# holuca/NeuralVolumetricReconstructionForMedicalImages

Measured on AMD Instinct MI355X. Metric: train rays/sec, chest 256^3 / 50 proj, higher is better.
Workload: dtype bf16; 1 GPU; chest_50.yaml: 256^3 volume, 50 cone-beam projections 512x512, hash L=16 T=2^19 C=2 (bf16 table), S=192, MLP 32-32-32-(64)-32-1, Adam lr 0.001; 1024 rays/step/GPU (reference n_rays=1024) = 1024 distinct valid pixels from one projection, drawn on the device inside the step; perturb=True; loss: chunk_sum (sum of 200-ray chunk means); the operating point that reaches 35 dB volume PSNR soonest (psnr.*; n_samples=192, parallelism=dp1

## Files before the change

include/naf_hip.h:

```cpp
#ifndef NAF_HIP_H
#define NAF_HIP_H

#include <stddef.h>
#include <stdint.h>

#ifdef __cplusplus
extern "C" {
#endif

typedef enum naf_status {
    NAF_OK = 0,
    NAF_ERR_INVALID_ARGUMENT = -1,
    NAF_ERR_UNSUPPORTED = -2,
    NAF_ERR_LAUNCH = -3
} naf_status;

typedef enum naf_dtype { NAF_F32 = 0, NAF_F16 = 1, NAF_BF16 = 2 } naf_dtype;

typedef enum naf_layout {
    NAF_LAYOUT_LBC = 0,
    NAF_LAYOUT_BLC = 1
} naf_layout;

const char *naf_last_error(void);
// ... 57 lines not shown
    float bound;
    uint32_t L, C, H;
    int32_t table_dtype;
    int32_t mlp_precision;
    int32_t last_activation;
    uint64_t seed;
    uint32_t ray_index_base;
    uint32_t log2_hashmap_size;
    int32_t scatter_mode;
    uint32_t flags;
} naf_render_cfg;

#define NAF_SCATTER_AUTO 0
#define NAF_SCATTER_ATOMIC 1
#define NAF_SCATTER_BINNED 2

#define NAF_CFG_PER_LEVEL_LAUNCHES 1u
#define NAF_CFG_EXPLICIT_DEPTHS 2u
#define NAF_CFG_LEVELS_INTERLEAVED 4u

#define NAF_CFG_FORWARD_FUSED 8u
#define NAF_CFG_ENCODE_TWO_GATHERS 32u
#define NAF_CFG_BACKWARD_ONE_WAVE_PER_SIMD 128u
#define NAF_CFG_ENCODE_LEVEL_MAJOR 256u
#define NAF_CFG_ENCODE_WINDOWS 64u
#define NAF_CFG_FUSED_STORE_FEATURES 16u
#define NAF_CFG_ENCODE_GROUPS_2 512u
#define NAF_CFG_ENCODE_GROUPS_4 1024u
#define NAF_CFG_MIN_BUCKETS_SHIFT 13u
#define NAF_CFG_MIN_BUCKETS_MASK (3u << NAF_CFG_MIN_BUCKETS_SHIFT)
#define NAF_CFG_SCATTER_PAIR12 2048u
#define NAF_CFG_LEVELS_GATHER_PASS 32768u
#define NAF_CFG_MLP_TWO_KERNELS 65536u
#define NAF_CFG_TEST_TINY_BLOCKS 4096u


int naf_scatter_overflow_count(const naf_render_cfg *cfg, uint64_t n_points, const void *workspace, uint32_t *count_host);

int naf_scatter_overflow_levels(const naf_render_cfg *cfg, uint64_t n_points, const void *workspace, uint32_t *counts_host);

size_t naf_render_workspace_bytes(const naf_render_cfg *cfg, uint64_t n_points);

size_t naf_forward_workspace_bytes(const naf_render_cfg *cfg, uint64_t n_points);

int naf_render_forward(const float *rays, const float *t_rand, const void *embeddings, const int32_t *offsets,
                       const float *mlp, float *acc, uint32_t n_rays, const naf_render_cfg *cfg, void *workspace,
                       void *stream);

int naf_render_forward_samples(const float *rays, const float *t_rand, const void *embeddings, const int32_t *offsets,
                               const float *mlp, float *acc, float *sigma, float *optical_depth, uint32_t n_rays,
                               const naf_render_cfg *cfg, void *workspace, void *stream);

int naf_render_backward(const float *rays, const float *t_rand, const float *grad_acc, const void *embeddings,
                        const int32_t *offsets, const float *mlp, float *grad_embeddings, float *grad_mlp, uint32_t n_rays,
                        const naf_render_cfg *cfg, void *workspace, int features_valid, void *stream);

int naf_render_train(const float *rays, const float *t_rand, const float *target, const float *ray_weight,
                     const void *embeddings, const int32_t *offsets, const float *mlp, float *acc,
                     float *grad_embeddings, float *grad_mlp, float *loss_out, uint32_t n_rays,
                     const naf_render_cfg *cfg, void *workspace, void *stream);

#define NAF_MAX_GRAD_BUCKETS 16
typedef struct naf_grad_buckets {
    uint32_t n_buckets;
    uint32_t level_begin[NAF_MAX_GRAD_BUCKETS];
    uint32_t level_end[NAF_MAX_GRAD_BUCKETS];
// ... 83 lines not shown
```

neuralvolumetricreconstructionformedicalimages_amd/_abi.py:

```python
from __future__ import annotations

import ctypes
import os

import torch

from . import build as _build

F32, F16, BF16 = 0, 1, 2
LAYOUT_LBC, LAYOUT_BLC = 0, 1
MLP_PARAMS = 4225
SCATTER_AUTO, SCATTER_ATOMIC, SCATTER_BINNED = 0, 1, 2
CFG_PER_LEVEL_LAUNCHES = 1
CFG_EXPLICIT_DEPTHS = 2
CFG_LEVELS_INTERLEAVED = 4
CFG_FORWARD_FUSED = 8
CFG_FUSED_STORE_FEATURES = 16
CFG_ENCODE_TWO_GATHERS = 32
CFG_ENCODE_WINDOWS = 64
CFG_BACKWARD_ONE_WAVE_PER_SIMD = 128
CFG_ENCODE_LEVEL_MAJOR = 256
CFG_ENCODE_GROUPS_2 = 512
CFG_ENCODE_GROUPS_4 = 1024
CFG_SCATTER_PAIR12 = 2048
CFG_TEST_TINY_BLOCKS = 4096
CFG_LEVELS_GATHER_PASS = 32768
CFG_MLP_TWO_KERNELS = 65536
CFG_MIN_BUCKETS_SHIFT = 13
GRAD_INPUTS_NONE, GRAD_INPUTS_EXACT, GRAD_INPUTS_REFERENCE = 0, 1, 2

_DTYPE_CODE = {torch.float32: F32, torch.float16: F16, torch.bfloat16: BF16}
_lib = None


class RenderCfg(ctypes.Structure):
    _fields_ = [
        ("n_samples", ctypes.c_uint32), ("perturb", ctypes.c_int32), ("bound", ctypes.c_float),
        ("L", ctypes.c_uint32), ("C", ctypes.c_uint32), ("H", ctypes.c_uint32),
        ("table_dtype", ctypes.c_int32), ("mlp_precision", ctypes.c_int32), ("last_activation", ctypes.c_int32),
        ("seed", ctypes.c_uint64), ("ray_index_base", ctypes.c_uint32), ("log2_hashmap_size", ctypes.c_uint32),
        ("scatter_mode", ctypes.c_int32), ("flags", ctypes.c_uint32),
    ]


MAX_GRAD_BUCKETS = 16


class GradBuckets(ctypes.Structure):
    _fields_ = [
        ("n_buckets", ctypes.c_uint32), ("level_begin", ctypes.c_uint32 * MAX_GRAD_BUCKETS),
        ("level_end", ctypes.c_uint32 * MAX_GRAD_BUCKETS), ("ready", ctypes.c_void_p * MAX_GRAD_BUCKETS),
        ("mlp_ready", ctypes.c_void_p),
    ]


MAX_DRAW_SEGMENTS = 16


class TableAdam(ctypes.Structure):
    _fields_ = [
# ... 150 lines not shown
```

neuralvolumetricreconstructionformedicalimages_amd/csrc/render_fused.hip:

```cpp
#include <algorithm>
#include <cmath>
#include <cstdio>
#include <cstring>
#include <type_traits>

#include "naf_host.h"
#include "hash_kernels.h"
#include "encode_kernel.h"
#include "field_mlp.h"
#include "field_mlp16.h"
#include "fused_forward.h"
#include "mlp_slabs.h"
#include "scatter_binned.h"
#include "scatter_v2.h"
#include "scatter_host.h"

namespace naf {

template <uint32_t kBytes> struct RawWord;
template <> struct RawWord<2> { typedef uint16_t type; };
template <> struct RawWord<4> { typedef uint32_t type; };
template <> struct RawWord<8> { typedef uint2 type; };
template <> struct RawWord<16> { typedef uint4 type; };

// ... 1107 lines not shown
    if (int rc = check_launch("mlp_backward_kernel")) return rc;
    if (ex.after_backward != nullptr && hipEventRecord(ex.after_backward, s) != hipSuccess) return fail(NAF_ERR_LAUNCH, "mlp backward: cannot record the event");
    return run_mlp_grad_reduce(slabs, grid, grad_mlp, loss_out, with_loss, madam, gmax_bits, ex, s);
}

static bool adam_tail_possible(const naf_render_cfg *cfg, const Workspace &w, uint32_t lv_begin, uint32_t lv_end) {
    if (!w.binned || per_level_launches(cfg)) return false;
    const uint32_t NB = 1u << w.plan.log2_nb;
    for (uint32_t l0 = lv_begin; l0 < lv_end; l0 += w.plan.levels_per_pass)
        if (reducer_split(NB, std::min(w.plan.levels_per_pass, lv_end - l0)) != 1u) return false;
    return true;
}

#ifndef NAF_V2_LV_FEW
#define NAF_V2_LV_FEW 4u
#endif
struct FxRecords {
    using Rec = PairFx;
    static constexpr uint32_t kThreads = 512u, kPoints = 2u, kLvMany = 16u, kLvFew = NAF_V2_LV_FEW;
    static constexpr bool kHasBig = true;
    const SrcRays &src;
    const void *dfeat;
    uint32_t B;
    DrawJob *next_draw;
    const GradBlocks *from_blocks;

    template <bool kFromBlocks>
    static auto bin_kernel_of(bool big, bool nb64, bool many) {
        constexpr uint32_t NT = kThreads;
        return big ? (many ? scatter_bin2_kernel<2u * NT, kLvMany, 0u, kFromBlocks> : scatter_bin2_kernel<2u * NT, kLvFew, 0u, kFromBlocks>)
                   : nb64 ? (many ? scatter_bin2_kernel<NT, kLvMany, 6u, kFromBlocks> : scatter_bin2_kernel<NT, kLvFew, 6u, kFromBlocks>)
                          : (many ? scatter_bin2_kernel<NT, kLvMany, 0u, kFromBlocks> : scatter_bin2_kernel<NT, kLvFew, 0u, kFromBlocks>);
    }
    auto bin_kernel(const BinPlan &plan, bool big, bool many) const {
        const bool nb64 = plan.log2_nb == 6u;
        return from_blocks != nullptr ? bin_kernel_of<true>(big, nb64, many) : bin_kernel_of<false>(big, nb64, many);
    }
    auto reduce_kernel(const AdamTail *adam) const {
        const bool fast = adam != nullptr && adam->lp != nullptr;
        return adam == nullptr ? scatter_reduce2_kernel<false, false> : fast ? scatter_reduce2_kernel<true, true> : scatter_reduce2_kernel<true, false>;
    }
    uint32_t bin_lds(const BinPlan &plan) const {
        return (3u * (1u << plan.log2_nb) + 4u) * 4u + (plan.slots + 1u) * (uint32_t)sizeof(PairFx) + side_list_capacity(plan.slots) * 12u;
    }
    template <typename K>
    void launch_bin(K bin, dim3 grid, uint32_t threads, uint32_t lds, hipStream_t s, const BinPass &p) const {
        DrawJob dj{};
        if (next_draw != nullptr && next_draw->count != 0u) { dj = *next_draw; next_draw->count = 0u; }
        grid.x += (dj.count + threads - 1u) / threads;
        const GradBlocks gb = from_blocks != nullptr ? *from_blocks : GradBlocks{};
        hipLaunchKernelGGL(bin, grid, dim3(threads), lds, s, src, (const uint16_t *)dfeat, p.offsets, p.grad_table, (PairFx *)p.w.regions,
                           p.w.counts, p.w.overflow, B, p.H, p.l0, p.nl, p.plan, p.job, dj, gb);
    }
};

template <typename P, uint32_t C>
static int run_hash_backward_levels(const SrcRays &src, const void *dfeat, const int32_t *offsets, float *grad_table, uint32_t B,
                                    const naf_render_cfg *cfg, const Workspace &w, uint32_t lv_begin, uint32_t lv_end, hipStream_t s,
                                    const naf_grad_buckets *buckets = nullptr, const AdamTail *adam = nullptr, const SlabReduce *slab_job = nullptr,
                                    DrawJob *next_draw = nullptr, const GradBlocks *from_blocks = nullptr) {
    using FT = typename P::feat_t;
    if (from_blocks != nullptr && !(w.binned && scatter_v2(cfg))) return fail(NAF_ERR_LAUNCH, "hash backward: only the 8-byte-record scatter reads gradient blocks in place");
    if (w.binned) {
        if (scatter_v2(cfg)) {
            FxRecords fam{src, dfeat, B, next_draw, from_blocks};
            return launch_binned_scatter(fam, cfg, w.plan, w.bin, offsets, grad_table, lv_begin, lv_end, buckets, s, adam, slab_job);
        }
        if (cfg->mlp_precision == NAF_F32) {
            PairRecords<FT, C, SrcRays, PairF32<C>, 16u, true> fam{src, dfeat, B, B, 1u};
            return launch_binned_scatter(fam, cfg, w.plan, w.bin, offsets, grad_table, lv_begin, lv_end, buckets, s, adam, slab_job);
        }
        PairRecords<FT, C, SrcRays, PairBF16<C>, 16u, true> fam{src, dfeat, B, B, 1u};
        return launch_binned_scatter(fam, cfg, w.plan, w.bin, offsets, grad_table, lv_begin, lv_end, buckets, s, adam, slab_job);
    }
    if (adam != nullptr) return fail(NAF_ERR_LAUNCH, "hash backward: the Adam tail needs the binned scatter");
    if (per_level_launches(cfg)) {
        static const char *const names[32] = NAF_LEVEL_NAMES("hash_backward_kernel_L");
        for (uint32_t l = lv_begin; l < lv_end; ++l) {
            ProfScope prof_(level_name(names, l), s);
            hipLaunchKernelGGL((hash_backward_kernel<FT, 3, C, SrcRays>), dim3(hash_grid_x(B), 1), dim3(256), 0, s, src,
                               (const typename FT::store_t *)dfeat, offsets, grad_table, B, cfg->L, cfg->H, false, l);
        }
        return check_launch("hash_backward_kernel");
    }
    { ProfScope prof_("hash_backward_kernel", s); hipLaunchKernelGGL((hash_backward_kernel<FT, 3, C, SrcRays>), dim3(hash_grid_x(B), lv_end - lv_begin), dim3(256), 0, s, src,
// ... 238 lines not shown
    const uint32_t units = vec ? run / (uint32_t)(16u / sizeof(T)) : run;
    const uint32_t gx = std::max<uint32_t>(1u, std::min<uint32_t>((units + 1023u) / 1024u, std::max<uint32_t>(1u, 512u / (n_ranks * nl))));
    {
        ProfScope prof_("levels_gather_kernel", s);
        if (vec) hipLaunchKernelGGL((levels_gather_kernel<T, true>), dim3(gx, n_ranks * nl), dim3(256), 0, s, (const unsigned char *)blocks, block_stride, (T *)w.dfeat, n_ranks, nl, run, lv_begin, gmax);
        else hipLaunchKernelGGL((levels_gather_kernel<T, false>), dim3(gx, n_ranks * nl), dim3(256), 0, s, (const unsigned char *)blocks, block_stride, (T *)w.dfeat, n_ranks, nl, run, lv_begin, gmax);
    }
    if (int rc = check_launch("levels_gather_kernel")) return rc;
    return run_hash_backward_levels<P, C>(src, w.dfeat, offsets, grad_emb, B, cfg, w, lv_begin, lv_end, s, nullptr, fuse ? &tail : nullptr, nullptr);
}

#define NAF_DISPATCH_PC(FN, ...)                                                                      \
    do {                                                                                              \
        if (cfg->mlp_precision == NAF_F32) {                                                          \
            switch (cfg->C) {                                                                         \
                case 1: return FN<PrecF32, 1>(__VA_ARGS__);                                           \
                case 2: return FN<PrecF32, 2>(__VA_ARGS__);                                           \
                case 4: return FN<PrecF32, 4>(__VA_ARGS__);                                           \
                default: return FN<PrecF32, 8>(__VA_ARGS__);                                          \
            }                                                                                         \
        }                                                                                             \
        switch (cfg->C) {                                                                             \
            case 1: return FN<PrecBF16, 1>(__VA_ARGS__);                                              \
            case 2: return FN<PrecBF16, 2>(__VA_ARGS__);                                              \
            case 4: return FN<PrecBF16, 4>(__VA_ARGS__);                                              \
            default: return FN<PrecBF16, 8>(__VA_ARGS__);                                             \
        }                                                                                             \
    } while (0)

}

using namespace naf;

#ifdef NAF_REDUCE_STAMPS
extern "C" int naf_debug_reduce_stamps(uint32_t *host, uint32_t n_words) {
    return hipMemcpyFromSymbol(host, HIP_SYMBOL(naf::g_reduce_stamps), (size_t)std::min<uint32_t>(n_words, 2048u * 8u) * 4u) == hipSuccess ? 0 : 1;
}
#endif

extern "C" int naf_scatter_overflow_count(const naf_render_cfg *cfg, uint64_t n_points, const void *workspace, uint32_t *count_host) {
    if (!cfg || !workspace || !count_host) return fail(NAF_ERR_INVALID_ARGUMENT, "scatter_overflow_count: null pointer");
    const Workspace w = carve(const_cast<void *>(workspace), cfg, n_points);
    *count_host = 0;
    if (!w.binned) return NAF_OK;
    if (hipMemcpy(count_host, w.bin.overflow, 4, hipMemcpyDeviceToHost) != hipSuccess) return fail(NAF_ERR_LAUNCH, "scatter_overflow_count: copy failed");
    return NAF_OK;
}

extern "C" int naf_scatter_overflow_levels(const naf_render_cfg *cfg, uint64_t n_points, const void *workspace, uint32_t *counts_host) {
    if (!cfg || !workspace || !counts_host) return fail(NAF_ERR_INVALID_ARGUMENT, "scatter_overflow_levels: null pointer");
    const Workspace w = carve(const_cast<void *>(workspace), cfg, n_points);
    std::memset(counts_host, 0, 32 * sizeof(uint32_t));
    if (!w.binned) return NAF_OK;
    if (hipMemcpy(counts_host, w.bin.overflow + 1, 32 * 4, hipMemcpyDeviceToHost) != hipSuccess) return fail(NAF_ERR_LAUNCH, "scatter_overflow_levels: copy failed");
    return NAF_OK;
}

extern "C" size_t naf_render_workspace_bytes(const naf_render_cfg *cfg, uint64_t n_points) {
    if (!cfg) return 0;
    return carve(nullptr, cfg, n_points).bytes;
}

extern "C" size_t naf_forward_workspace_bytes(const naf_render_cfg *cfg, uint64_t n_points) {
    if (!cfg) return 0;
    return forward_workspace_bytes(cfg, n_points);
}
// ... 273 lines not shown
```

neuralvolumetricreconstructionformedicalimages_amd/csrc/scatter_host.h:

```cpp
#pragma once

#include <algorithm>

#include "naf_host.h"
#include "scatter_binned.h"
#include "scatter_v2.h"

namespace naf {

static inline bool per_level_launches(const naf_render_cfg *cfg) { return (cfg->flags & NAF_CFG_PER_LEVEL_LAUNCHES) != 0u; }

constexpr uint64_t kBinMinPoints = 1u << 13;
constexpr size_t kBinBudgetBytes = (size_t)40 << 30;

static inline bool scatter_v2(const naf_render_cfg *cfg) {
    return cfg->mlp_precision == NAF_BF16 && cfg->C == 2u && (cfg->flags & NAF_CFG_SCATTER_PAIR12) == 0u;
}
static inline size_t record_bytes(const naf_render_cfg *cfg) {
    if (scatter_v2(cfg)) return sizeof(PairFx);
    return cfg->mlp_precision == NAF_F32 ? 4u * (1u + 2u * cfg->C) : 4u * (1u + 2u * ((cfg->C + 1u) / 2u));
}
static inline uint32_t bin_threads(const naf_render_cfg *cfg) { return record_bytes(cfg) <= 12 ? 512u : 256u; }
static inline uint32_t bin_points_per_thread(const naf_render_cfg *cfg) { return record_bytes(cfg) <= 20 ? 2u : 1u; }
constexpr uint32_t kBigTileLog2Nb = 7u;
// ... 17 lines not shown
    if ((cfg->flags & NAF_CFG_TEST_TINY_BLOCKS) != 0u) plan->slots = std::max(32u, tile & ~31u);
    const uint32_t mean_run = std::max<uint32_t>(1u, (tile * 4u) >> log2_nb);
    plan->log2_w = 3u;
    while (plan->log2_w < 6u && (1u << plan->log2_w) < mean_run + mean_run / 4u) ++plan->log2_w;
    plan->max_local_rows = (uint32_t)((((maxT + (1ull << log2_nb) - 1) >> log2_nb) + 63u) & ~63ull);
    const size_t per_level = (size_t)plan->n_tiles * plan->slots * rec;
    plan->levels_per_pass = (uint32_t)std::min<size_t>(cfg->L, std::max<size_t>(1, kBinBudgetBytes / per_level));
    if (per_level_launches(cfg)) plan->levels_per_pass = 1;
    return true;
}

static inline uint32_t reducer_split(uint32_t NB, uint32_t nl) { return NB * nl >= 256u ? 1u : std::max(1u, std::min(16u, 1024u / (NB * nl))); }

struct BinRegions {
    unsigned char *regions;
    uint32_t *counts;
    uint32_t *overflow;
    uint32_t *gmax;
    size_t bytes;
};

static inline BinRegions carve_bin_regions(unsigned char *base, const naf_render_cfg *cfg, const BinPlan &plan) {
    const size_t n_runs = ((size_t)plan.levels_per_pass << plan.log2_nb) * plan.n_tiles;
    const size_t block_bytes = ((size_t)plan.levels_per_pass * plan.n_tiles * plan.slots * record_bytes(cfg) + 255) & ~(size_t)255;
    BinRegions r;
    r.regions = base;
    r.counts = (uint32_t *)(base + block_bytes);
    r.overflow = r.counts + n_runs;
    r.gmax = r.overflow + 33;
    r.bytes = block_bytes + (((n_runs + 33 + 1) * 4 + 255) & ~(size_t)255);
    return r;
}

struct BinPass {
    const int32_t *offsets;
    float *grad_table;
    const BinRegions &w;
    uint32_t H, l0, nl;
    const BinPlan &plan;
    const SlabReduce &job;
};

template <typename F>
static int launch_binned_scatter(F &fam, const naf_render_cfg *cfg, const BinPlan &plan, const BinRegions &w, const int32_t *offsets,
                                 float *grad_table, uint32_t lv_begin, uint32_t lv_end, const naf_grad_buckets *buckets, hipStream_t s,
                                 const AdamTail *adam = nullptr, const SlabReduce *slab_job = nullptr) {
    constexpr uint32_t NT = F::kThreads, PTS = F::kPoints;
    const bool big = F::kHasBig && plan.tile_points == 2u * NT * PTS;
    if (!big && plan.tile_points != NT * PTS) return fail(NAF_ERR_LAUNCH, "binned scatter: plan / kernel tile mismatch");
    const uint32_t threads = big ? 2u * NT : NT;
    const bool many = plan.n_tiles >= (big ? 768u : 1536u);
    const uint32_t LV = many ? F::kLvMany : F::kLvFew;
    const auto bin = fam.bin_kernel(plan, big, many);
    const auto red = fam.reduce_kernel(adam);
    const AdamTail tail = adam != nullptr ? *adam : AdamTail{};
    const uint32_t NB = 1u << plan.log2_nb;
    const uint32_t red_lds = plan.max_local_rows * cfg->C * 8u, bin_lds = fam.bin_lds(plan);
    if (int rc = raise_lds_limit(red, red_lds, "binned scatter: cannot raise dynamic LDS limit (reduce)")) return rc;
    if (int rc = raise_lds_limit(bin, bin_lds, "binned scatter: cannot raise dynamic LDS limit (bin)")) return rc;
    static const char *const bin_names[32] = NAF_LEVEL_NAMES("scatter_bin_kernel_L");
    static const char *const red_names[32] = NAF_LEVEL_NAMES("scatter_reduce_kernel_L");
    const bool per_level = per_level_launches(cfg);
    SlabReduce job{};
    if (slab_job != nullptr) job = *slab_job;
    auto launch_bin = [&](uint32_t l0, uint32_t nl) -> int {
        ProfScope prof_(per_level ? level_name(bin_names, l0) : "scatter_bin_kernel", s);
        const uint32_t spare = job.slabs != nullptr ? kSlabReduceBlocks : 0u;
        fam.launch_bin(bin, dim3(plan.n_tiles + spare, (nl + LV - 1u) / LV), threads, bin_lds, s, BinPass{offsets, grad_table, w, cfg->H, l0, nl, plan, job});
        job = SlabReduce{};
        return check_launch("scatter_bin_kernel");
    };
    auto launch_reduce = [&](uint32_t l0, uint32_t ly0, uint32_t nl) -> int {
        ProfScope prof_(per_level ? level_name(red_names, l0 + ly0) : "scatter_reduce_kernel", s);
        const uint32_t n_split = reducer_split(NB, nl);
        if (adam != nullptr && n_split != 1u) return fail(NAF_ERR_LAUNCH, "binned scatter: the Adam tail needs unsplit reducer launches");
        hipLaunchKernelGGL(red, dim3(NB, nl, n_split), dim3(1024), red_lds, s, (const typename F::Rec *)w.regions, w.counts, offsets,
                           grad_table, w.gmax, l0, ly0, cfg->H, plan, tail);
        return check_launch("scatter_reduce_kernel");
    };
    if (buckets != nullptr && !per_level && plan.levels_per_pass >= cfg->L && lv_begin == 0u && lv_end == cfg->L) {
        if (int rc = launch_bin(0u, cfg->L)) return rc;
        for (uint32_t b = 0; b < buckets->n_buckets; ++b) {
            if (int rc = launch_reduce(0u, buckets->level_begin[b], buckets->level_end[b] - buckets->level_begin[b])) return rc;
            if (buckets->ready[b] != nullptr && hipEventRecord((hipEvent_t)buckets->ready[b], s) != hipSuccess)
                return fail(NAF_ERR_LAUNCH, "render_train: cannot record a bucket event");
        }
        return NAF_OK;
    }
    for (uint32_t l0 = lv_begin; l0 < lv_end; l0 += plan.levels_per_pass) {
        const uint32_t nl = std::min(plan.levels_per_pass, lv_end - l0);
        if (int rc = launch_bin(l0, nl)) return rc;
        if (int rc = launch_reduce(l0, 0u, nl)) return rc;
    }
    return NAF_OK;
}

template <typename FT, uint32_t C, typename Src, typename R, uint32_t kLvMany_, bool kAdamTail>
struct PairRecords {
    using Rec = R;
    static constexpr uint32_t kThreads = BinShape<Rec>::kThreads, kPoints = BinShape<Rec>::kPoints, kLvMany = kLvMany_, kLvFew = 4u;
    static constexpr bool kHasBig = sizeof(Rec) <= 12;
    Src src;
    const void *grad;
    uint32_t B, sl, sb;

    auto bin_kernel(const BinPlan &, bool big, bool many) const {
        constexpr uint32_t NT = kThreads, PTS = kPoints;
        auto bin = many ? scatter_bin_kernel<FT, C, Src, Rec, NT, PTS, kLvMany> : scatter_bin_kernel<FT, C, Src, Rec, NT, PTS, kLvFew>;
        if constexpr (kHasBig) {
            if (big) bin = many ? scatter_bin_kernel<FT, C, Src, Rec, 2u * NT, PTS, kLvMany> : scatter_bin_kernel<FT, C, Src, Rec, 2u * NT, PTS, kLvFew>;
        }
        return bin;
    }
    auto reduce_kernel(const AdamTail *adam) const {
        if constexpr (kAdamTail) { if (adam != nullptr) return scatter_reduce_kernel<C, Rec, true>; }
        return scatter_reduce_kernel<C, Rec, false>;
    }
    uint32_t bin_lds(const BinPlan &plan) const { return (2u * (1u << plan.log2_nb) + 4u) * 4u + plan.slots * (uint32_t)sizeof(Rec); }
    template <typename K>
    void launch_bin(K bin, dim3 grid, uint32_t threads, uint32_t lds, hipStream_t s, const BinPass &p) const {
        hipLaunchKernelGGL(bin, grid, dim3(threads), lds, s, src, (const typename FT::store_t *)grad, p.offsets, p.grad_table, (Rec *)p.w.regions,
                           p.w.counts, p.w.overflow, B, p.H, p.l0, p.nl, p.plan, p.job, sl, sb);
    }
};

}
```

neuralvolumetricreconstructionformedicalimages_amd/csrc/scatter_v2.h:

```cpp
#pragma once

#include "draw_device.h"
#include "hash_kernels.h"
#include "scatter_binned.h"

namespace naf {

struct __attribute__((aligned(8))) PairFx {
    uint32_t head, pay;
};
constexpr uint32_t kFxLocalBits = 13u, kFxBits = 15u;
constexpr uint32_t kFxEShift = kFxLocalBits, kFxShift = kFxLocalBits + 4u;
constexpr int kFixHead2 = 26;

__device__ __forceinline__ int fixed_shift2(uint32_t gmax_bits) {
    const int e = (int)((gmax_bits >> 23) & 0xffu);
    if (e == 0 || e == 255) return 0;
    const int s = kFixHead2 - (e - 127) - 1;
    return s > 120 ? 120 : s;
}

__device__ __forceinline__ uint32_t pack_bf16x2(float lo, float hi) {
    typedef __bf16 bf16x2 __attribute__((ext_vector_type(2)));
    bf16x2 pk;
// ... 22 lines not shown
    v += (uint32_t)__builtin_amdgcn_update_dpp(0, (int)v, 0x111, 0xf, 0xf, false);
    v += (uint32_t)__builtin_amdgcn_update_dpp(0, (int)v, 0x112, 0xf, 0xf, false);
    v += (uint32_t)__builtin_amdgcn_update_dpp(0, (int)v, 0x114, 0xf, 0xf, false);
    v += (uint32_t)__builtin_amdgcn_update_dpp(0, (int)v, 0x118, 0xf, 0xf, false);
    v += (uint32_t)__builtin_amdgcn_update_dpp(0, (int)v, 0x142, 0xa, 0xf, false);
    v += (uint32_t)__builtin_amdgcn_update_dpp(0, (int)v, 0x143, 0xc, 0xf, false);
    return v;
}

__device__ __forceinline__ uint32_t wave_max_to_lane63(uint32_t v) {
    v = max(v, (uint32_t)__builtin_amdgcn_update_dpp(0, (int)v, 0x111, 0xf, 0xf, false));
    v = max(v, (uint32_t)__builtin_amdgcn_update_dpp(0, (int)v, 0x112, 0xf, 0xf, false));
    v = max(v, (uint32_t)__builtin_amdgcn_update_dpp(0, (int)v, 0x114, 0xf, 0xf, false));
    v = max(v, (uint32_t)__builtin_amdgcn_update_dpp(0, (int)v, 0x118, 0xf, 0xf, false));
    v = max(v, (uint32_t)__builtin_amdgcn_update_dpp(0, (int)v, 0x142, 0xa, 0xf, false));
    v = max(v, (uint32_t)__builtin_amdgcn_update_dpp(0, (int)v, 0x143, 0xc, 0xf, false));
    return v;
}

struct GradBlocks {
    uint32_t rank_points;
    uint32_t block_points;
    uint32_t level0;
    uint32_t magic, shift;
    uint32_t *gmax_bits;
};
static inline GradBlocks make_grad_blocks(uint32_t rank_points, uint32_t block_points, uint32_t level0, uint32_t *gmax_bits) {
    uint32_t l = 0;
    while ((1ull << l) < rank_points) ++l;
    const uint64_t two = 1ull << (31u + l);
    return GradBlocks{rank_points, block_points, level0, (uint32_t)((two + rank_points - 1u) / rank_points), l - 1u, gmax_bits};
}

template <uint32_t NT, uint32_t LV, uint32_t kLog2NB, bool kFromBlocks = false>
__global__ void __launch_bounds__(NT, 4)
scatter_bin2_kernel(SrcRays src, const uint16_t *__restrict__ grad, const int32_t *__restrict__ offsets, float *__restrict__ grad_table,
                    PairFx *__restrict__ blocks, uint32_t *__restrict__ runs, uint32_t *__restrict__ overflow, uint32_t B, uint32_t H,
                    uint32_t level_base, uint32_t n_levels, BinPlan plan, SlabReduce slab_job, DrawJob draw_job, GradBlocks gb = GradBlocks{}) {
    extern __shared__ __attribute__((aligned(16))) unsigned char smem[];
    if (blockIdx.x >= plan.n_tiles) {
        if (blockIdx.y == 0u) {
            const uint32_t spare = blockIdx.x - plan.n_tiles, n_slab = slab_job.slabs != nullptr ? kSlabReduceBlocks : 0u;
            if (spare < n_slab) slab_reduce_block<NT / kReduceParams>(reinterpret_cast<float (*)[kReduceParams]>(smem), slab_job, spare, threadIdx.x);
            else {
                const uint32_t t = (spare - n_slab) * NT + threadIdx.x;
                if (t < draw_job.count) draw_one(draw_job, t);
            }
        }
        return;
    }
    constexpr uint32_t PTS = 2u;
    constexpr bool kWaveScan = kLog2NB == 6u;
    const uint32_t log2_nb = kLog2NB != 0u ? kLog2NB : plan.log2_nb, NB = 1u << log2_nb, nb_mask = NB - 1u, SLOTS = plan.slots;
    uint32_t *hist = reinterpret_cast<uint32_t *>(smem);
    uint32_t *start = hist + 2u * NB;
    uint32_t *misc = start + NB;
    uint2 *staging = reinterpret_cast<uint2 *>(misc + 4);
    const uint32_t side_cap = side_list_capacity(SLOTS);
    uint32_t *side = reinterpret_cast<uint32_t *>(staging + SLOTS + 1u);
    const uint32_t tile = blockIdx.x, lane = threadIdx.x & 63u, wave = __builtin_amdgcn_readfirstlane(threadIdx.x >> 6);
    for (uint32_t i = threadIdx.x; i < 2u * NB; i += NT) hist[i] = 0u;
    if (threadIdx.x < 4u) misc[threadIdx.x] = 0u;
    uint32_t published = 0u;
    if constexpr (kFromBlocks) {
        if (threadIdx.x == 3u) { published = __hip_atomic_load(gb.gmax_bits, __ATOMIC_RELAXED, __HIP_MEMORY_SCOPE_AGENT); misc[3] = published; }
    }

    float x[PTS][3];
    uint32_t bp[PTS];
    bool valid[PTS];
#pragma unroll
    for (uint32_t q = 0; q < PTS; ++q) {
        const uint32_t b_raw = (tile * PTS + q) * NT + threadIdx.x;
        valid[q] = b_raw < B;
        bp[q] = valid[q] ? b_raw : B - 1u;
        src.get(bp[q], x[q]);
    }
    const float spacing = src.sample_spacing();
    if constexpr (kFromBlocks) {
#pragma unroll
        for (uint32_t q = 0; q < PTS; ++q) {
            const uint32_t r = __umulhi(bp[q], gb.magic) >> gb.shift;
            bp[q] += r * (gb.block_points - gb.rank_points);
        }
    }
    auto grad_at = [&](uint32_t level, uint32_t q) __attribute__((always_inline)) -> uint32_t {
        if constexpr (kFromBlocks) return *reinterpret_cast<const uint32_t *>(grad + ((size_t)(level - gb.level0) * gb.rank_points + bp[q]) * 2u);
        else return *reinterpret_cast<const uint32_t *>(grad + ((size_t)level * B + bp[q]) * 2u);
    };
    uint32_t graw[PTS];
    uint32_t wmax = 0u;
    if (blockIdx.y * LV < n_levels) {
#pragma unroll
        for (uint32_t q = 0; q < PTS; ++q) graw[q] = grad_at(level_base + blockIdx.y * LV, q);
    }
    __syncthreads();
    if constexpr (kFromBlocks) wmax = (uint32_t)__builtin_amdgcn_readfirstlane((int)misc[3]);
    const uint32_t seed = (uint32_t)__builtin_amdgcn_readlane((int)published, 3);
    uint32_t n_overflow = 0, n_overflow_level = 0;

    for (uint32_t it = 0; it < LV; ++it) {
        const uint32_t ly = blockIdx.y * LV + it;
        if (ly >= n_levels) break;
        const uint32_t level = level_base + ly, cur = it & 1u;
        uint32_t *hist_c = hist + cur * NB, *side_n = misc + 1u + cur;
        const LevelMeta m = make_level_meta<3>(offsets, level, H);
        float *__restrict__ gg = grad_table + (size_t)m.offset * 2u;
        const RowMap map = make_row_map(m.mode, m.size, log2_nb);
        const bool merging = m.scale * spacing < 0.5f && m.scale < 65535.0f;
        const bool fast = !merging && bucket_shift(m.size, 0u) <= map.hs;

#ifndef NAF_DIAG_BLOCKS_NO_MAX
        if constexpr (kFromBlocks) {
            uint32_t gm = 0u;
#pragma unroll
            for (uint32_t q = 0; q < PTS; ++q) gm = max(gm, max((graw[q] << 16) & 0x7fffffffu, graw[q] & 0x7fff0000u));
            if (__ballot(gm > wmax) != 0ull) {
                wmax = (uint32_t)__builtin_amdgcn_readlane((int)wave_max_to_lane63(gm), 63);
                if (lane == 0u) atomicMax(&misc[3], wmax);
            }
        }
#endif
        uint32_t head[PTS][4], pay[PTS][4], bkt[PTS][4], rank[PTS][4];
        bool on[PTS];
        auto emit_b = [&](uint32_t rb, uint32_t p) __attribute__((always_inline)) {
            const uint32_t i = atomicAdd(side_n, 1u);
            if (i < side_cap) {
                const uint32_t b = map.bucket(rb, nb_mask), r = atomicAdd(&hist_c[b], 1u);
                side[3u * i] = (b << 16) | r; side[3u * i + 1u] = map.local(rb); side[3u * i + 2u] = p;
            } else {
                spill_record(gg, rb, 0u, p);
                ++n_overflow;
                ++n_overflow_level;
            }
        };
#pragma unroll
// ... 92 lines not shown
                }
                if (__ballot(any) != 0ull) {
#pragma unroll
                    for (uint32_t k = 0; k < 4; ++k) {
                        if (single[k]) {
                            const float wyz = wy[k & 1u] * wz[k >> 1];
                            const float p0 = wyz * g[0], p1 = wyz * g[1];
                            head[q][k] &= (1u << kFxLocalBits) - 1u; pay[q][k] = pack_bf16x2(p0 * gx, p1 * gx);
                            emit_b(ra[k] ^ xm[k], pack_bf16x2(p0 * fx, p1 * fx));
                        }
                    }
                }
            }
            if (merging && __ballot(merged_lane) != 0ull) {
#pragma unroll
                for (uint32_t k = 0; k < 4; ++k) {
                    if (merged_lane) {
                        head[q][k] &= (1u << kFxLocalBits) - 1u; pay[q][k] = pack_bf16x2(va[k][0], va[k][1]);
                        emit_b(ra[k] ^ xm[k], pack_bf16x2(vb[k][0], vb[k][1]));
                    }
                }
            }
            if (fast) {
#pragma unroll
                for (uint32_t k = 0; k < 4; ++k) rank[q][k] = atomicAdd(&hist_c[bkt[q][k]], 1u);
            } else {
#pragma unroll
                for (uint32_t k = 0; k < 4; ++k) {
                    rank[q][k] = 0u;
                    if (on[q]) rank[q][k] = atomicAdd(&hist_c[bkt[q][k]], 1u);
                }
            }
        }
        if (it + 1u < LV && ly + 1u < n_levels) {
#pragma unroll
            for (uint32_t q = 0; q < PTS; ++q) graw[q] = grad_at(level + 1u, q);
        }
        lds_barrier();
#pragma unroll
        for (uint32_t q = 0; q < PTS; ++q) asm volatile("" : "+v"(graw[q]) : : "memory");
#ifndef NAF_DIAG_BLOCKS_NO_TAIL
        if constexpr (kFromBlocks) {
            if ((it + 1u == LV || ly + 1u == n_levels) && threadIdx.x == 0u) {
                const uint32_t m = misc[3];
                if (m > seed) atomicMax(gb.gmax_bits, m);
            }
        }
#endif

        if (wave == 0u) {
            for (uint32_t i = lane; i < NB; i += 64u) hist[(cur ^ 1u) * NB + i] = 0u;
            if (lane == 0u) misc[1u + (cur ^ 1u)] = 0u;
        }
        uint32_t excl = 0u, total = 0u;
        if constexpr (kWaveScan) {
            const uint32_t n = hist_c[lane];
            const uint32_t incl = wave_inclusive_sum(n);
            excl = incl - n;
            total = (uint32_t)__builtin_amdgcn_readlane((int)incl, 63);
            if (wave == 0u) {
                const uint32_t start_c = min(excl, SLOTS), n_c = min(n, SLOTS - start_c);
                runs[run_index(plan, ly, lane, tile)] = start_c | (n_c << 16);
            }
        } else {
            if (wave == 0u) {
                const uint32_t per = NB >> 6;
                uint32_t mine = 0u;
// ... 61 lines not shown
            for (uint32_t q = 0; q < PTS; ++q)
#pragma unroll
                for (uint32_t k = 0; k < 4; ++k) {
                    const uint32_t pos = offset_of(bkt[q][k]) + rank[q][k];
                    if ((fast || on[q]) && pos >= SLOTS) {
                        spill_record(gg, map.row(bkt[q][k], head[q][k] & ((1u << kFxLocalBits) - 1u)), head[q][k], pay[q][k]);
                        ++n_overflow;
                        ++n_overflow_level;
                    }
                }
        }
        lds_barrier();

        {
            const uint32_t n_rec = min(total, SLOTS);
            const uint32_t n_chunk = min(((n_rec * 8u + 127u) >> 7) << 3, (SLOTS * 8u) >> 4);
            typedef uint32_t u32x4 __attribute__((ext_vector_type(4)));
            u32x4 *__restrict__ dst = reinterpret_cast<u32x4 *>(blocks + block_index(plan, ly, tile));
            const u32x4 *from = reinterpret_cast<const u32x4 *>(staging);
            for (uint32_t c = threadIdx.x; c < n_chunk; c += NT) __builtin_nontemporal_store(from[c], dst + c);
        }
        if (__ballot(n_overflow_level != 0u)) {
#pragma unroll
            for (int off = 32; off > 0; off >>= 1) n_overflow_level += __shfl_xor(n_overflow_level, off, 64);
            if (lane == 0u) atomicAdd(overflow + 1u + level, n_overflow_level);
            n_overflow_level = 0u;
        }
    }
    if (__ballot(n_overflow != 0u)) {
#pragma unroll
        for (int off = 32; off > 0; off >>= 1) n_overflow += __shfl_xor(n_overflow, off, 64);
        if (lane == 0u) atomicAdd(overflow, n_overflow);
    }
}

__device__ __forceinline__ int cvt_rpi(float v) {
    int i;
    asm("v_cvt_rpi_i32_f32 %0, %1" : "=v"(i) : "v"(v));
    return i;
}

__device__ __forceinline__ PairFx load_record(const PairFx *p) {
#ifdef NAF_V2_NT_LOADS
    typedef uint32_t u32x2 __attribute__((ext_vector_type(2)));
    const u32x2 v = __builtin_nontemporal_load(reinterpret_cast<const u32x2 *>(p));
    return PairFx{v.x, v.y};
#else
    return *p;
#endif
}

#ifdef NAF_REDUCE_STAMPS
__device__ uint32_t g_reduce_stamps[2048 * 8];
#define NAF_RSTAMP(i) rs_[i] = clock64()
#else
#define NAF_RSTAMP(i)
#endif

template <bool kAdam, bool kFast>
__global__ void __launch_bounds__(1024)
scatter_reduce2_kernel(const PairFx *__restrict__ blocks, const uint32_t *__restrict__ runs, const int32_t *__restrict__ offsets,
                       float *__restrict__ grad_table, const uint32_t *__restrict__ gmax_bits, uint32_t level_base, uint32_t ly_begin,
                       uint32_t H, BinPlan plan, AdamTail adam) {
    extern __shared__ __attribute__((aligned(16))) unsigned char smem[];
#ifdef NAF_REDUCE_STAMPS
    long long rs_[5] = {0, 0, 0, 0, 0};
// ... 280 lines not shown
```

Before: 4.591 million rays/s.

## Flatten scatter-bin grid into balanced tile-level work items per resident group

Adds a flat variant of the binned scatter kernel that splits tile×level work items evenly across a grid sized to a multiple of twice the CU count, instead of a 2D tile × level-chunk grid. Each workgroup walks consecutive (tile, level) items, reloading ray positions when it wraps to the next tile, and prefetches the next gradient accordingly. This targets load imbalance and tail effects when there are few tiles with 64 buckets. A flag disables it. It also adds optional debug timestamp instrumentation.

```diff
diff --git a/include/naf_hip.h b/include/naf_hip.h
--- a/include/naf_hip.h
+++ b/include/naf_hip.h
@@ -113,6 +113,7 @@
 #define NAF_CFG_SCATTER_PAIR12 2048u
 #define NAF_CFG_LEVELS_GATHER_PASS 32768u
 #define NAF_CFG_MLP_TWO_KERNELS 65536u
+#define NAF_CFG_SCATTER_BIN_TILE_GRID 131072u
 #define NAF_CFG_TEST_TINY_BLOCKS 4096u
 
 
diff --git a/neuralvolumetricreconstructionformedicalimages_amd/_abi.py b/neuralvolumetricreconstructionformedicalimages_amd/_abi.py
--- a/neuralvolumetricreconstructionformedicalimages_amd/_abi.py
+++ b/neuralvolumetricreconstructionformedicalimages_amd/_abi.py
@@ -26,6 +26,7 @@
 CFG_TEST_TINY_BLOCKS = 4096
 CFG_LEVELS_GATHER_PASS = 32768
 CFG_MLP_TWO_KERNELS = 65536
+CFG_SCATTER_BIN_TILE_GRID = 131072
 CFG_MIN_BUCKETS_SHIFT = 13
 GRAD_INPUTS_NONE, GRAD_INPUTS_EXACT, GRAD_INPUTS_REFERENCE = 0, 1, 2
 
diff --git a/neuralvolumetricreconstructionformedicalimages_amd/csrc/render_fused.hip b/neuralvolumetricreconstructionformedicalimages_amd/csrc/render_fused.hip
--- a/neuralvolumetricreconstructionformedicalimages_amd/csrc/render_fused.hip
+++ b/neuralvolumetricreconstructionformedicalimages_amd/csrc/render_fused.hip
@@ -1163,8 +1163,10 @@
                    : nb64 ? (many ? scatter_bin2_kernel<NT, kLvMany, 6u, kFromBlocks> : scatter_bin2_kernel<NT, kLvFew, 6u, kFromBlocks>)
                           : (many ? scatter_bin2_kernel<NT, kLvMany, 0u, kFromBlocks> : scatter_bin2_kernel<NT, kLvFew, 0u, kFromBlocks>);
     }
-    auto bin_kernel(const BinPlan &plan, bool big, bool many) const {
+    bool flat_bin(const BinPlan &plan, bool big) const { return !big && plan.log2_nb == 6u && from_blocks == nullptr; }
+    auto bin_kernel(const BinPlan &plan, bool big, bool many, bool flat) const {
         const bool nb64 = plan.log2_nb == 6u;
+        if (flat) return scatter_bin2_kernel<kThreads, kLvFew, 6u, false, true>;
         return from_blocks != nullptr ? bin_kernel_of<true>(big, nb64, many) : bin_kernel_of<false>(big, nb64, many);
     }
     auto reduce_kernel(const AdamTail *adam) const {
@@ -1181,7 +1183,7 @@
         grid.x += (dj.count + threads - 1u) / threads;
         const GradBlocks gb = from_blocks != nullptr ? *from_blocks : GradBlocks{};
         hipLaunchKernelGGL(bin, grid, dim3(threads), lds, s, src, (const uint16_t *)dfeat, p.offsets, p.grad_table, (PairFx *)p.w.regions,
-                           p.w.counts, p.w.overflow, B, p.H, p.l0, p.nl, p.plan, p.job, dj, gb);
+                           p.w.counts, p.w.overflow, B, p.H, p.l0, p.nl, p.plan, p.job, dj, gb, p.groups);
     }
 };
 
@@ -1486,6 +1488,11 @@
 
 using namespace naf;
 
+#ifdef NAF_BIN_STAMPS
+extern "C" int naf_debug_bin_stamps(uint32_t *host, uint32_t n_words) {
+    return hipMemcpyFromSymbol(host, HIP_SYMBOL(naf::g_bin_stamps), (size_t)std::min<uint32_t>(n_words, naf::kBinStampGroups * 8u) * 4u) == hipSuccess ? 0 : 1;
+}
+#endif
 #ifdef NAF_REDUCE_STAMPS
 extern "C" int naf_debug_reduce_stamps(uint32_t *host, uint32_t n_words) {
     return hipMemcpyFromSymbol(host, HIP_SYMBOL(naf::g_reduce_stamps), (size_t)std::min<uint32_t>(n_words, 2048u * 8u) * 4u) == hipSuccess ? 0 : 1;
diff --git a/neuralvolumetricreconstructionformedicalimages_amd/csrc/scatter_host.h b/neuralvolumetricreconstructionformedicalimages_amd/csrc/scatter_host.h
--- a/neuralvolumetricreconstructionformedicalimages_amd/csrc/scatter_host.h
+++ b/neuralvolumetricreconstructionformedicalimages_amd/csrc/scatter_host.h
@@ -73,6 +73,22 @@
     return r;
 }
 
+static inline uint32_t resident_bin_groups() {
+    static int cus[64] = {};
+    int dev = 0;
+    if (hipGetDevice(&dev) != hipSuccess || dev < 0 || dev >= 64) dev = 0;
+    if (cus[dev] == 0) {
+        int n = 0;
+        cus[dev] = hipDeviceGetAttribute(&n, hipDeviceAttributeMultiprocessorCount, dev) == hipSuccess && n > 0 ? n : 1;
+    }
+    return 2u * (uint32_t)cus[dev];
+}
+
+static inline uint32_t flat_bin_groups(uint32_t n_items, uint32_t resident) {
+    const uint32_t half = n_items / 2u;
+    return half >= resident ? half / resident * resident : std::max(1u, half);
+}
+
 struct BinPass {
     const int32_t *offsets;
     float *grad_table;
@@ -80,6 +96,7 @@
     uint32_t H, l0, nl;
     const BinPlan &plan;
     const SlabReduce &job;
+    uint32_t groups;
 };
 
 template <typename F>
@@ -92,7 +109,9 @@
     const uint32_t threads = big ? 2u * NT : NT;
     const bool many = plan.n_tiles >= (big ? 768u : 1536u);
     const uint32_t LV = many ? F::kLvMany : F::kLvFew;
-    const auto bin = fam.bin_kernel(plan, big, many);
+    const bool per_level = per_level_launches(cfg);
+    const bool flat = !many && !per_level && (cfg->flags & NAF_CFG_SCATTER_BIN_TILE_GRID) == 0u && fam.flat_bin(plan, big);
+    const auto bin = fam.bin_kernel(plan, big, many, flat);
     const auto red = fam.reduce_kernel(adam);
     const AdamTail tail = adam != nullptr ? *adam : AdamTail{};
     const uint32_t NB = 1u << plan.log2_nb;
@@ -101,13 +120,14 @@
     if (int rc = raise_lds_limit(bin, bin_lds, "binned scatter: cannot raise dynamic LDS limit (bin)")) return rc;
     static const char *const bin_names[32] = NAF_LEVEL_NAMES("scatter_bin_kernel_L");
     static const char *const red_names[32] = NAF_LEVEL_NAMES("scatter_reduce_kernel_L");
-    const bool per_level = per_level_launches(cfg);
     SlabReduce job{};
     if (slab_job != nullptr) job = *slab_job;
     auto launch_bin = [&](uint32_t l0, uint32_t nl) -> int {
         ProfScope prof_(per_level ? level_name(bin_names, l0) : "scatter_bin_kernel", s);
         const uint32_t spare = job.slabs != nullptr ? kSlabReduceBlocks : 0u;
-        fam.launch_bin(bin, dim3(plan.n_tiles + spare, (nl + LV - 1u) / LV), threads, bin_lds, s, BinPass{offsets, grad_table, w, cfg->H, l0, nl, plan, job});
+        const uint32_t groups = flat ? flat_bin_groups(plan.n_tiles * nl, resident_bin_groups()) : 0u;
+        const dim3 grid = flat ? dim3(groups + spare, 1u) : dim3(plan.n_tiles + spare, (nl + LV - 1u) / LV);
+        fam.launch_bin(bin, grid, threads, bin_lds, s, BinPass{offsets, grad_table, w, cfg->H, l0, nl, plan, job, groups});
         job = SlabReduce{};
         return check_launch("scatter_bin_kernel");
     };
@@ -145,7 +165,8 @@
     const void *grad;
     uint32_t B, sl, sb;
 
-    auto bin_kernel(const BinPlan &, bool big, bool many) const {
+    bool flat_bin(const BinPlan &, bool) const { return false; }
+    auto bin_kernel(const BinPlan &, bool big, bool many, bool) const {
         constexpr uint32_t NT = kThreads, PTS = kPoints;
         auto bin = many ? scatter_bin_kernel<FT, C, Src, Rec, NT, PTS, kLvMany> : scatter_bin_kernel<FT, C, Src, Rec, NT, PTS, kLvFew>;
         if constexpr (kHasBig) {
diff --git a/neuralvolumetricreconstructionformedicalimages_amd/csrc/scatter_v2.h b/neuralvolumetricreconstructionformedicalimages_amd/csrc/scatter_v2.h
--- a/neuralvolumetricreconstructionformedicalimages_amd/csrc/scatter_v2.h
+++ b/neuralvolumetricreconstructionformedicalimages_amd/csrc/scatter_v2.h
@@ -78,15 +78,29 @@
     return GradBlocks{rank_points, block_points, level0, (uint32_t)((two + rank_points - 1u) / rank_points), l - 1u, gmax_bits};
 }
 
-template <uint32_t NT, uint32_t LV, uint32_t kLog2NB, bool kFromBlocks = false>
+#ifdef NAF_BIN_STAMPS
+constexpr uint32_t kBinStampGroups = 4096u;
+__device__ uint32_t g_bin_stamps[kBinStampGroups * 8u];
+__device__ __forceinline__ void bin_stamp(uint32_t wall0, uint32_t first_ly, uint32_t n_items) {
+    if (threadIdx.x != 0u) return;
+    uint32_t *dbg = g_bin_stamps + ((blockIdx.y * gridDim.x + blockIdx.x) & (kBinStampGroups - 1u)) * 8u;
+    dbg[0] = wall0; dbg[1] = (uint32_t)wall_clock64();
+    dbg[2] = __builtin_amdgcn_s_getreg((31 << 11) | 4); dbg[3] = __builtin_amdgcn_s_getreg((3 << 11) | 20);
+    dbg[4] = blockIdx.x; dbg[5] = blockIdx.y; dbg[6] = first_ly; dbg[7] = n_items + 1u;
+}
+#endif
+
+template <uint32_t NT, uint32_t LV, uint32_t kLog2NB, bool kFromBlocks = false, bool kFlat = false>
 __global__ void __launch_bounds__(NT, 4)
 scatter_bin2_kernel(SrcRays src, const uint16_t *__restrict__ grad, const int32_t *__restrict__ offsets, float *__restrict__ grad_table,
                     PairFx *__restrict__ blocks, uint32_t *__restrict__ runs, uint32_t *__restrict__ overflow, uint32_t B, uint32_t H,
-                    uint32_t level_base, uint32_t n_levels, BinPlan plan, SlabReduce slab_job, DrawJob draw_job, GradBlocks gb = GradBlocks{}) {
+                    uint32_t level_base, uint32_t n_levels, BinPlan plan, SlabReduce slab_job, DrawJob draw_job, GradBlocks gb = GradBlocks{}, uint32_t n_groups = 0u) {
+    static_assert(!(kFlat && kFromBlocks), "the level-parallel path publishes its maximum by level order inside a workgroup");
     extern __shared__ __attribute__((aligned(16))) unsigned char smem[];
-    if (blockIdx.x >= plan.n_tiles) {
+    const uint32_t n_bin = kFlat ? n_groups : plan.n_tiles;
+    if (blockIdx.x >= n_bin) {
         if (blockIdx.y == 0u) {
-            const uint32_t spare = blockIdx.x - plan.n_tiles, n_slab = slab_job.slabs != nullptr ? kSlabReduceBlocks : 0u;
+            const uint32_t spare = blockIdx.x - n_bin, n_slab = slab_job.slabs != nullptr ? kSlabReduceBlocks : 0u;
             if (spare < n_slab) slab_reduce_block<NT / kReduceParams>(reinterpret_cast<float (*)[kReduceParams]>(smem), slab_job, spare, threadIdx.x);
             else {
                 const uint32_t t = (spare - n_slab) * NT + threadIdx.x;
@@ -104,7 +118,21 @@
     uint2 *staging = reinterpret_cast<uint2 *>(misc + 4);
     const uint32_t side_cap = side_list_capacity(SLOTS);
     uint32_t *side = reinterpret_cast<uint32_t *>(staging + SLOTS + 1u);
-    const uint32_t tile = blockIdx.x, lane = threadIdx.x & 63u, wave = __builtin_amdgcn_readfirstlane(threadIdx.x >> 6);
+#ifdef NAF_BIN_STAMPS
+    const uint32_t bwall_ = (uint32_t)wall_clock64();
+#endif
+    uint32_t tile = blockIdx.x, ly_f = 0u, n_it = LV;
+    if constexpr (kFlat) {
+        const uint32_t n_items = plan.n_tiles * n_levels;
+        const uint32_t i0 = (uint32_t)(((uint64_t)blockIdx.x * n_items) / n_groups), i1 = (uint32_t)(((uint64_t)(blockIdx.x + 1u) * n_items) / n_groups);
+        tile = i0 / n_levels;
+        ly_f = i0 - tile * n_levels;
+        n_it = i1 - i0;
+    }
+#ifdef NAF_BIN_STAMPS
+    const uint32_t bfirst_ = kFlat ? ly_f : blockIdx.y * LV;
+#endif
+    const uint32_t lane = threadIdx.x & 63u, wave = __builtin_amdgcn_readfirstlane(threadIdx.x >> 6);
     for (uint32_t i = threadIdx.x; i < 2u * NB; i += NT) hist[i] = 0u;
     if (threadIdx.x < 4u) misc[threadIdx.x] = 0u;
     uint32_t published = 0u;
@@ -115,13 +143,16 @@
     float x[PTS][3];
     uint32_t bp[PTS];
     bool valid[PTS];
-#pragma unroll
-    for (uint32_t q = 0; q < PTS; ++q) {
-        const uint32_t b_raw = (tile * PTS + q) * NT + threadIdx.x;
-        valid[q] = b_raw < B;
-        bp[q] = valid[q] ? b_raw : B - 1u;
-        src.get(bp[q], x[q]);
-    }
+    auto locate_tile = [&]() __attribute__((always_inline)) {
+#pragma unroll
+        for (uint32_t q = 0; q < PTS; ++q) {
+            const uint32_t b_raw = (tile * PTS + q) * NT + threadIdx.x;
+            valid[q] = b_raw < B;
+            bp[q] = valid[q] ? b_raw : B - 1u;
+            src.get(bp[q], x[q]);
+        }
+    };
+    locate_tile();
     const float spacing = src.sample_spacing();
     if constexpr (kFromBlocks) {
 #pragma unroll
@@ -136,7 +167,12 @@
     };
     uint32_t graw[PTS];
     uint32_t wmax = 0u;
-    if (blockIdx.y * LV < n_levels) {
+    if constexpr (kFlat) {
+        if (n_it != 0u) {
+#pragma unroll
+            for (uint32_t q = 0; q < PTS; ++q) graw[q] = grad_at(level_base + ly_f, q);
+        }
+    } else if (blockIdx.y * LV < n_levels) {
 #pragma unroll
         for (uint32_t q = 0; q < PTS; ++q) graw[q] = grad_at(level_base + blockIdx.y * LV, q);
     }
@@ -145,9 +181,16 @@
     const uint32_t seed = (uint32_t)__builtin_amdgcn_readlane((int)published, 3);
     uint32_t n_overflow = 0, n_overflow_level = 0;
 
-    for (uint32_t it = 0; it < LV; ++it) {
-        const uint32_t ly = blockIdx.y * LV + it;
-        if (ly >= n_levels) break;
+    for (uint32_t it = 0; it < n_it; ++it) {
+        if constexpr (kFlat) {
+            if (it != 0u && ++ly_f == n_levels) {
+                ly_f = 0u;
+                ++tile;
+                locate_tile();
+            }
+        }
+        const uint32_t ly = kFlat ? ly_f : blockIdx.y * LV + it;
+        if (!kFlat && ly >= n_levels) break;
         const uint32_t level = level_base + ly, cur = it & 1u;
         uint32_t *hist_c = hist + cur * NB, *side_n = misc + 1u + cur;
         const LevelMeta m = make_level_meta<3>(offsets, level, H);
@@ -306,7 +349,16 @@
                 }
             }
         }
-        if (it + 1u < LV && ly + 1u < n_levels) {
+        if constexpr (kFlat) {
+            if (it + 1u < n_it) {
+                const bool wrap = ly + 1u == n_levels;
+#pragma unroll
+                for (uint32_t q = 0; q < PTS; ++q) {
+                    const uint32_t b_next = wrap ? min(bp[q] + PTS * NT, B - 1u) : bp[q];
+                    graw[q] = *reinterpret_cast<const uint32_t *>(grad + ((size_t)(wrap ? level_base : level + 1u) * B + b_next) * 2u);
+                }
+            }
+        } else if (it + 1u < LV && ly + 1u < n_levels) {
 #pragma unroll
             for (uint32_t q = 0; q < PTS; ++q) graw[q] = grad_at(level + 1u, q);
         }
@@ -434,6 +486,9 @@
         for (int off = 32; off > 0; off >>= 1) n_overflow += __shfl_xor(n_overflow, off, 64);
         if (lane == 0u) atomicAdd(overflow, n_overflow);
     }
+#ifdef NAF_BIN_STAMPS
+    bin_stamp(bwall_, bfirst_, kFlat ? n_it : min(LV, n_levels - min(n_levels, blockIdx.y * LV)));
+#endif
 }
 
 __device__ __forceinline__ int cvt_rpi(float v) {
```

Result: slower. 4.352 million rays/s (-5.2%).
